# jankammeth/BA-path-planning

Hardware: AMD Instinct MI355X
Metric: SCP iterations/sec (N agents x K waypoints) (higher is better)
Workload: dtype f64

## Files before the change

ba-path-planning_amd/csrc/scp_qp.hip:

```cpp
#include "scp_qp_internal.h"
#include "scp_reset_device.h"

#include <chrono>
#include <cmath>
#include <vector>

__global__ __launch_bounds__(256) void qp_reset_kernel(int N, int K, int D, int Rf, const double* __restrict__ x0,
                                                        const double* __restrict__ F, const double* __restrict__ S0,
                                                        double* __restrict__ x, double* __restrict__ zf,
                                                        double* __restrict__ fx, double* __restrict__ Qx,
                                                        double* __restrict__ yf) {
  extern __shared__ double reset_xs[];
  qp_reset_body<false>(threadIdx.x, true, reset_xs, N, K, D, Rf, x0, F, S0, x, zf, fx, Qx, yf);
}

namespace {

inline size_t align_up(size_t v, size_t a = 256) { return (v + a - 1) / a * a; }

struct Carver {
  char* base;
  size_t off;
  template <typename T>
  T* take(size_t count) {
// ... 46 lines not shown
  d.s0p = c.take<double>(nx);
  d.fx = c.take<double>(nf);
  d.dyf = c.take<double>(nf);
  d.dyc = c.take<double>((size_t)cap);
  const size_t ncell = (size_t)(C / D) * K;
  d.cell_ptr = c.take<int>(ncell + 1);
  d.cell_cur = c.take<int>(ncell);
  d.scan_tot = c.take<int>(ncell / 4096 + 2);
  d.ent_code = c.take<int>((size_t)2 * cap);
  d.coef = c.take<double>((size_t)2 * cap * D);
  d.gval = c.take<double>((size_t)2 * cap);
  d.gval2 = c.take<double>((size_t)2 * cap);
  d.gval3 = c.take<double>((size_t)2 * cap);
  d.pos_i = c.take<int>((size_t)cap);
  d.pos_j = c.take<int>((size_t)cap);
  d.sync_words = c.take<unsigned long long>(SCP_SYNC_WORDS);
  d.cells = c.take<unsigned long long>((size_t)2 * nx);
  d.gpart = c.take<unsigned long long>(SCP_GPART_WORDS);
  d.gcheck = c.take<unsigned long long>(SCP_GCHECK_WORDS);
  return c.off;
}

}

extern "C" void scp_qp_default_settings(scp_qp_settings* s) {
  if (!s) return;
  s->rho = 0.1;
  s->sigma = 1e-6;
  s->alpha = 1.6;
  s->rho_eq_scale = 1e3;
// ... 45 lines not shown
  qp->st = *s;
  qp->row_cap = row_capacity;
  qp->nW = 0;
  qp->problem_set = qp->reset_done = false;
  qp->rho = s->rho;
  carve(qp->d, workspace, K, qp->C, row_capacity, D);
  scp_qp_kkt_init_slots(qp);
  qp->check_seq = 0;
  qp->persist_off = false;
  qp->persist_skip_solve = false;
  qp->persist_gave_up_total = 0;
  qp->persist_variant = 0;
  qp->steps_since_reset = 0;
  memset(qp->lim, 0, sizeof(qp->lim));
  qp->persist_fault = 0;
  qp->persist_cap_nW = -1;
  qp->persist_cap = 0;
  qp->persist_epoch = 0;
  if (hipHostMalloc(&qp->h_scal, (SL_COUNT + SCP_RESID_CAP + 4) * sizeof(double),
                    hipHostMallocMapped | hipHostMallocCoherent) != hipSuccess ||
      hipHostGetDevicePointer((void**)&qp->h_scal_dev, qp->h_scal, 0) != hipSuccess) {
    delete qp;
    return scp_fail(ctx, SCP_ERR_HIP, "qp_create: hipHostMalloc failed");
  }
  memset(qp->h_scal, 0, (SL_COUNT + SCP_RESID_CAP + 4) * sizeof(double));
  qp->h_persist = (unsigned*)(qp->h_scal + SL_COUNT + SCP_RESID_CAP + 1);
  qp->h_persist_dev = (unsigned*)(qp->h_scal_dev + SL_COUNT + SCP_RESID_CAP + 1);
  const int Rf = qp->Rf;
  std::vector<double> F((size_t)Rf * K, 0.0), Ft((size_t)Rf * K, 0.0), S0((size_t)K * K, 0.0), S0t((size_t)K * K, 0.0),
      w(Rf, 1.0);
// ... 406 lines not shown
  if (y_col && qp->nW > 0)
    SCP_HIP_CHECK(ctx, hipMemcpyAsync(y_col, qp->d.yc, qp->nW * sizeof(double), hipMemcpyDeviceToDevice, ctx->stream));
  return SCP_OK;
}

extern "C" int scp_qp_peek(scp_qp* qp, const char* name, double* out, int64_t cap, int64_t* n_out) {
  if (!qp) return SCP_ERR_INVALID;
  scp_ctx* ctx = qp->ctx;
  SCP_REQUIRE(ctx, name && out && n_out, "qp_peek: null pointer");
  const QpDev& d = qp->d;
  const int64_t nf = (int64_t)qp->Rf * qp->C, nx = (int64_t)qp->K * qp->C;
  const double* src = nullptr;
  int64_t n = 0;
  if (!strcmp(name, "fx")) { src = d.fx; n = nf; }
  else if (!strcmp(name, "qx")) { src = scp_qp_qx(qp); n = nx; }
  else if (!strcmp(name, "gval")) { src = d.gval; n = 2 * qp->nW; }
  else if (!strcmp(name, "zf")) { src = d.zf; n = nf; }
  else if (!strcmp(name, "yf")) { src = d.yf; n = nf; }
  else if (!strcmp(name, "zc")) { src = d.zc; n = qp->nW; }
  else if (!strcmp(name, "yc")) { src = d.yc; n = qp->nW; }
  else if (!strcmp(name, "x")) { src = d.x; n = nx; }
  else if (!strcmp(name, "w_eta")) { src = d.w_eta; n = qp->nW * qp->D; }
  else if (!strcmp(name, "w_l")) { src = d.w_l; n = qp->nW; }
  else if (!strcmp(name, "p")) { src = d.p; n = nx; }
  else if (!strcmp(name, "qp")) { src = d.s0p; n = nx; }
  else if (!strcmp(name, "Hf")) { src = d.Hf; n = (int64_t)qp->K * qp->K; }
  else if (!strcmp(name, "Minv")) { src = d.Minv; n = (int64_t)qp->K * qp->K; }
  else if (!strcmp(name, "T")) { src = d.T; n = (int64_t)qp->K * qp->K; }
  else return scp_fail(ctx, SCP_ERR_INVALID, "qp_peek: unknown array %s", name);
  *n_out = n;
  if (n > cap) return scp_fail(ctx, SCP_ERR_CAPACITY, "qp_peek: %lld doubles needed", (long long)n);
  if (n > 0) SCP_HIP_CHECK(ctx, hipMemcpyAsync(out, src, (size_t)n * sizeof(double), hipMemcpyDeviceToDevice, ctx->stream));
  return SCP_OK;
}

extern "C" int scp_qp_debug_set(scp_qp* qp, const char* key, int value) {
  if (!qp || !key) return SCP_ERR_INVALID;
  if (!strcmp(key, "persist_fault")) {
    if (value >= 0) qp->persist_fault = value;
    return qp->persist_fault;
  }
  if (!strcmp(key, "persist_off")) {
    if (value >= 0) qp->persist_off = value != 0;
    return qp->persist_off ? 1 : 0;
  }
  if (!strcmp(key, "persist_gave_up_total")) return qp->persist_gave_up_total;
  return scp_fail(qp->ctx, SCP_ERR_INVALID, "qp_debug_set: unknown key %s", key);
}
```

ba-path-planning_amd/csrc/scp_qp_columns.hip:

```cpp
#include "scp_qp_device.h"

namespace {

using namespace scpdev;
constexpr int FT = 1024;
constexpr int NWV = FT / 64;

#ifdef SCP_PHASE_PROFILE
__device__ unsigned long long scp_phase_clk[64];
#define PHASE_MARK(slot)                                                                      \
  do {                                                                                        \
    if (blockIdx.x == gridDim.x / 2 && threadIdx.x == 0) scp_phase_clk[slot] = wall_clock64(); \
  } while (0)
#else
#define PHASE_MARK(slot) ((void)0)
#endif

constexpr int SQ_BLOCKS = 128;
template <int E>
__global__ __launch_bounds__(FT) void cg1_col_kernel(int K, int Rf, int64_t C, double rho, double h,
                                                      const double* __restrict__ pMinv, const double* __restrict__ wrow,
                                                      const double* __restrict__ x, const double* __restrict__ Fx,
                                                      const double* __restrict__ zf, const double* __restrict__ yf, int N,
                                                      int D, const int* __restrict__ cell_ptr,
// ... 586 lines not shown
  gval[posj] = g;
}

}

int scp_qp_qp0_iterations(scp_qp* qp, int nit, double* dy_out) {
  const QpDev& d = qp->d;
  const int K = qp->K, Rf = qp->Rf;
  const int nblk = (int)((qp->C + CB - 1) / CB);
  const size_t lds = (size_t)CB * (pad_col(Rf) + 3 * pad_col(K)) * sizeof(double);
  return qp_launch(qp, K <= 64 ? qp0_col_kernel<1> : qp0_col_kernel<2>, dim3(nblk), dim3(FT), lds, K, Rf, qp->C, qp->rho,
                   qp->st.sigma, qp->st.alpha, qp->h, nit, d.pMinv, d.wrow, d.lf, d.uf, d.x, d.zf, d.yf, dy_out);
}

int scp_qp_cg1_prepare(scp_qp* qp) {
  if (qp->dv.carried) return SCP_OK;
  QP_CHECK(scp_qp_exact_qx(qp, true));
  QP_CHECK(scp_qp_rows_first_values(qp, scp_qp_qx(qp)));
  qp_on_cg1_prepared(qp);
  return SCP_OK;
}

int scp_qp_cg1_iteration(scp_qp* qp, int* cg_count, bool emit_dy) {
  const QpDev& d = qp->d;
  double* dyf = emit_dy ? d.dyf : nullptr;
  double* dyc = emit_dy ? d.dyc : nullptr;
  const int K = qp->K, Rf = qp->Rf;
  const int64_t C = qp->C;
  const int nblk = (int)((C + CB - 1) / CB);
  double* Qp = d.s0p;
  double* Fp = d.tf;
// ... 314 lines not shown
```

ba-path-planning_amd/csrc/scp_qp_internal.h:

```cpp
#pragma once
#include "scp_common.h"

#define QP_CHECK(call)            \
  do {                            \
    int rc_ = (call);             \
    if (rc_ != SCP_OK) return rc_; \
  } while (0)

constexpr int SCP_KKT_SLOTS = 6;
constexpr int SCP_KKT_SLOTS_MAX = 32;
constexpr size_t SCP_KKT_POOL_BYTES = (size_t)48 << 20;
constexpr int SCP_INV_LDS_MAX_K = 96;
static inline size_t scp_packed_count(int R, int M) { return (size_t)((R + 15) / 16) * ((M + 3) / 4) * 64; }
size_t scp_qp_kkt_pool_doubles(int K);
void scp_qp_kkt_init_slots(scp_qp* qp);
int scp_qp_build_g0(scp_qp* qp);
int scp_qp_build_kkt(scp_qp* qp);

enum Slot {
  SL_RZ0 = 0, SL_RZ1 = 1,
  SL_RP = 8, SL_NAX = 9, SL_NZ = 10, SL_RD = 11, SL_NPX = 12, SL_NATY = 13,
  SL_NDY = 14, SL_SUPP = 15, SL_NATDY = 16,
  SL_COUNT = 32
};
// ... 14 lines not shown
  double* scal;
  double* part;
  double* s0p;
  double* fx;
  double* dyf;
  double* dyc;
  int* cell_ptr;
  int* cell_cur;
  int* scan_tot;
  int* ent_code;
  double* coef;
  double* gval;
  double* gval2;
  double* gval3;
  int *pos_i, *pos_j;
  double* kkt_pool;
  unsigned long long* sync_words;
  unsigned long long* cells;
  unsigned long long* gpart;
  unsigned long long* gcheck;
};

struct QpDerived {
  bool lists = false;
  bool qx = false;
  int qx_half = 0;
  double vals_rho_c = 0.0;
  bool carried = false;
};

struct scp_qp {
  scp_ctx* ctx;
  int N, K, D, Rf;
  int64_t C;
  double h;
  scp_qp_settings st;
  int64_t row_cap, nW;
  bool problem_set, reset_done;
  QpDerived dv;
  double rho;
  QpDev d;
  struct KktSlot {
    double rho, sigma;
    unsigned long long used;
    double *Hf, *HS, *Minv, *T, *pMinv, *pT;
  } kkt[SCP_KKT_SLOTS_MAX];
  int n_kkt;
  unsigned long long kkt_clock;
  double* h_scal;
  double* h_scal_dev;
  unsigned long long check_seq;
  double space[6];
  double lim[6];
  int64_t steps_since_reset;
  int persist_variant;
  int persist_fault;
  bool persist_off;
  bool persist_skip_solve;
  int persist_gave_up_total;
  int64_t persist_cap_nW;
  int persist_cap;
  unsigned long long persist_epoch;
  unsigned* h_persist;
  int persist_rho_switches;
  double persist_rho;
  unsigned* h_persist_dev;
};

constexpr int64_t SCP_FINE_MAX_COLUMNS = 4096;
inline int scp_qp_fine_cadence(const scp_qp* qp) {
  const scp_qp_settings& st = qp->st;
// ... 15 lines not shown
constexpr int NPART = 128;
int scp_qp_generic_iteration(scp_qp* qp, int* cg_count);
int scp_qp_generic_residuals(scp_qp* qp, bool with_dy);
int scp_qp_generic_certificate_atdy(scp_qp* qp);
int scp_qp_exact_qx(scp_qp* qp, bool with_fx);
inline double* scp_qp_qx(const scp_qp* qp, bool other = false) {
  return (qp->dv.qx_half != 0) != other ? qp->d.HQ : qp->d.HQ + (int64_t)qp->K * qp->C;
}

int scp_qp_append_rows(scp_qp* qp, int64_t n, const int64_t* rows, const double* eta, const double* l, int64_t eta_stride,
                       int64_t q_begin, int64_t nq, const double* Qx);
int scp_qp_csr_ensure(scp_qp* qp);
int scp_qp_csr_scatter(scp_qp* qp, int mode, const double* vec);
int scp_qp_rows_gather(scp_qp* qp, const double* Q);
int scp_qp_rows_first_values(scp_qp* qp, const double* Qx);
int scp_qp_rows_check_values(scp_qp* qp, bool with_dy);
int scp_qp_install_rows_small(scp_qp* qp, int64_t n, const int64_t* rows, const double* pos_prev, const double* p0,
                              const double* v0, double R, const double* Qx, bool* done);
int scp_qp_reset_install_small(scp_qp* qp, const double* x0, int64_t n, const int64_t* rows, const double* pos_prev,
                               const double* p0, const double* v0, double R, double* Qx, bool* done);

constexpr int SCP_RESID_STRIDE = 12;
constexpr int SCP_RESID_CAP = (4096 / 2 + 128) * SCP_RESID_STRIDE;
constexpr int SCP_BIGK_MAX_K = 1024;
constexpr int SCP_FUSED_MAX_K = 120;
constexpr int SCP_PART_CAP = 4096;
int scp_qp_cg1_iteration(scp_qp* qp, int* cg_count, bool emit_dy);
int scp_qp_qp0_iterations(scp_qp* qp, int nit, double* dy_out);
int scp_qp_cg1_prepare(scp_qp* qp);
int scp_qp_fused_residuals(scp_qp* qp, bool with_dy);

constexpr int SCP_SYNC_WORDS = 16;
constexpr int SCP_PERSIST_MAX_WG = 256;
constexpr int SCP_GPART_WORDS = 2 * (SCP_PERSIST_MAX_WG + 1) * 4;
constexpr int SCP_GCHECK_WORDS = (SCP_PERSIST_MAX_WG + 1) * 9 * 2;
bool scp_qp_persist_eligible(const scp_qp* qp);
bool scp_persist_claim(int device, int n_cu_total, int n_wg, int wait_ms);
void scp_persist_release(int device, int n_wg);
constexpr int SCP_PERSIST_GAVE_UP = 2;
int scp_qp_cg1_persist(scp_qp* qp, int it0, int cad0, int* ran, int* code, int* it_done);

inline void qp_on_x_set(scp_qp* qp, bool qx) {
  QpDerived& v = qp->dv;
  v.lists = v.carried = false; v.vals_rho_c = 0.0; v.qx = qx;
  if (qx) v.qx_half = 0;
}
inline void qp_on_rows_added(scp_qp* qp, bool small_install) {
  qp->dv.lists = small_install; qp->dv.vals_rho_c = small_install ? qp->rho * qp->st.rho_col_scale : 0.0;
  qp->dv.carried = false;
}
inline void qp_on_rho_changed(scp_qp* qp, bool in_kernel) { qp->dv.vals_rho_c = 0.0; qp->dv.carried &= in_kernel; }
inline void qp_on_solve_start(scp_qp* qp) { qp->dv.carried = false; }
inline void qp_on_scratch_used(scp_qp* qp) { qp->dv.carried = qp->dv.qx = false; qp->dv.vals_rho_c = 0.0; }
inline void qp_on_fused_check(scp_qp* qp) { qp->dv.qx = true; }
inline void qp_on_cg1_step(scp_qp* qp) { qp->dv.qx = false; qp->dv.qx_half ^= 1; }
inline void qp_on_persist_exit(scp_qp* qp, int code) {
  qp->dv.qx = code != SCP_PERSIST_GAVE_UP;
  if (code == SCP_PERSIST_GAVE_UP) qp->dv.carried = false;
}
inline void qp_on_qx_built(scp_qp* qp, bool with_fx) { qp->dv.qx_half = 0; qp->dv.qx = with_fx; }
inline void qp_on_lists_built(scp_qp* qp) { qp->dv.lists = true; }
inline void qp_on_cg1_prepared(scp_qp* qp) { qp->dv.lists = qp->dv.carried = true; qp->dv.vals_rho_c = 0.0; }
```

ba-path-planning_amd/csrc/scp_qp_persist.hip:

```cpp
#include "scp_qp_persist_device.h"

#include <algorithm>
#include <cstdlib>
#include <cerrno>
#include <chrono>


namespace {
using namespace scpdev;
using namespace scp_persist;

#ifdef SCP_PHASE_PROFILE
__device__ unsigned long long scp_persist_clk[16];
#define PSTAMP(slot)                                  \
  do {                                                \
    const unsigned long long now_ = wall_clock64();   \
    pacc[slot] += now_ - plast;                       \
    plast = now_;                                     \
  } while (0)
#else
#define PSTAMP(slot) ((void)0)
#endif

constexpr int persist_apb(int D) { return D == 3 ? 4 : CB / D; }
// ... 28 lines not shown
  int* cptr = e_row + cap;

  const int wave = threadIdx.x >> 6, lane = threadIdx.x & 63;
  const int a0 = blockIdx.x * APB;
  const int agent = a0 + wave;
  const bool aok = agent < N;
  const int k = lane;
  const bool live = aok && k < K;
  const double h = A.h, hh = h * h, alpha = A.alpha;
  double rho = A.rho, rho_c = A.rho_c;
  unsigned n_rho = 0;
  const int tK = (K + 15) >> 4, nks = (K + 3) >> 2;
  const int nblk = A.nblk;

  const int a1 = min(a0 + APB, N);
  const int ebase = A.cell_ptr[cell_of(0, a0, K)];
  const int ne = A.cell_ptr[cell_of(0, a1, K)] - ebase;
  if (entries_overflow<APB>(A)) return;
  if (threadIdx.x == 0) fail_s = 0;
  for (int i = threadIdx.x; i <= (a1 - a0) * K; i += NT) cptr[i] = A.cell_ptr[cell_of(0, a0, K) + i] - ebase;
  for (int e = threadIdx.x; e < ne; e += NT) {
    const int code = A.ent_code[ebase + e];
    const int n = code >> 1, side = code & 1;
    const int wi = A.w_i[n], wj = A.w_j[n], wk = A.w_k[n];
    const int own = side ? wj : wi, par = side ? wi : wj;
    e_code[e] = wk | ((own - a0) << 8) | (side << 16);
    e_pad[e] = ((wk * N + par) * D) * 2;
    e_row[e] = n;
    const int64_t bo = (int64_t)wk * C + (int64_t)own * D, bp = (int64_t)wk * C + (int64_t)par * D;
#pragma unroll
    for (int d = 0; d < D; ++d) {
      const double eta = A.w_eta[(size_t)n * D + d];
      e_c[(size_t)e * D + d] = side ? -eta : eta;
      e_qo[(size_t)e * D + d] = A.Qx[bo + d];
      e_qp[(size_t)e * D + d] = A.Qx[bp + d];
    }
    e_l[e] = A.w_l[n];
    e_z[e] = A.zc[n];
    e_y[e] = A.yc[n];
    e_g[e] = A.gval[ebase + e];
  }
  for (int i = threadIdx.x; i < CB * RSK; i += NT) Rt[i] = 0.0;

  double z[D][4], y[D][4], lo[D][4], hi[D][4], fx[D][4], rr[4], x[D], qx[D];
#pragma unroll
  for (int t = 0; t < 4; ++t) {
    const bool rok = live && (t > 0 || k < K - 1);
    const int row = t == 0 ? k : t * K - 1 + k;
    rr[t] = (t >= 2 && k == K - 1) ? rho * A.rho_eq : rho;
#pragma unroll
    for (int d = 0; d < D; ++d) {
      z[d][t] = y[d][t] = lo[d][t] = hi[d][t] = fx[d][t] = 0.0;
      if (rok) {
        const int64_t g = (int64_t)row * C + (int64_t)agent * D + d;
        z[d][t] = A.zf[g]; y[d][t] = A.yf[g]; lo[d][t] = A.lf[g]; hi[d][t] = A.uf[g]; fx[d][t] = A.fx[g];
// ... 353 lines not shown
        A.zf[g] = z[d][t];
        A.yf[g] = y[d][t];
        A.fx[g] = fx[d][t];
        if (with_dy) A.dyf[g] = dy[d][t];
      }
    }
  }
  if (live) {
#pragma unroll
    for (int d = 0; d < D; ++d) {
      const int64_t g = (int64_t)k * C + (int64_t)agent * D + d;
      A.x[g] = x[d];
      A.Qx[g] = qx[d];
    }
  }
  for (int e = threadIdx.x; e < ne; e += NT) {
    A.gval[ebase + e] = e_g[e];
    if (!((e_code[e] >> 16) & 1)) {
      A.zc[e_row[e]] = e_z[e];
      A.yc[e_row[e]] = e_y[e];
      if (with_dy) A.dyc[e_row[e]] = e_pp[(size_t)e * D];
    }
  }
  PSTAMP(8);
#ifdef SCP_PHASE_PROFILE
  if (blockIdx.x == gridDim.x / 2 && threadIdx.x == 0)
    for (int i = 0; i < 16; ++i) scp_persist_clk[i] = i == 15 ? (unsigned long long)steps : pacc[i];
#endif
  publish_exit(A, chk, it_done, n_rho, rho, exit_code);
}

size_t persist_lds_bytes(int K, int cap, int nblk, int D, int apb) {
  size_t dbl = (size_t)3 * CB * pad_col(K) + (size_t)apb * 64 * D + (size_t)NCHK * nblk + (size_t)cap * (4 * D + 4);
  size_t ints = (size_t)3 * cap + (size_t)apb * K + 1;
  return dbl * sizeof(double) + ((ints + 1) / 2 * 2) * sizeof(int);
// ... 36 lines not shown
}

int scp_qp_cg1_persist(scp_qp* qp, int it0, int cad0, int* ran, int* code, int* it_done) {
  const QpDev& d = qp->d;
  scp_ctx* ctx = qp->ctx;
  hipStream_t s = ctx->stream;
  const scp_qp_settings& st = qp->st;
  const int K = qp->K, D = qp->D;
  const int64_t C = qp->C;
  const int variant = persist_variant_for(qp);
  if (variant < 0) { *ran = 0; return SCP_OK; }
  const PersistKernel pk = persist_kernel(variant, D);
  const int apb = pk.apb;
  const int nblk = (qp->N + apb - 1) / apb;
  *ran = 0;
  QP_CHECK(scp_qp_cg1_prepare(qp));
  if (qp->persist_cap_nW == qp->nW) return SCP_OK;
  {
    const int nb = nblk + 1;
    const size_t fixed = pk.lds_bytes(K, 0, nb, D, apb);
    const size_t budget_lds = 160 * 1024 - pk.static_lds;
    if (fixed + 64 * pk.entry_bytes > budget_lds) return SCP_OK;
    qp->persist_cap = (int)((budget_lds - fixed) / pk.entry_bytes / 64 * 64);
  }
  const int nblk_expected = nblk + (qp->persist_fault > 0 ? 1 : 0);
  const size_t lds = pk.lds_bytes(K, qp->persist_cap, nblk_expected, D, apb);
  if (lds > 160 * 1024) return SCP_OK;
  const int budget = st.max_iter - it0;
  if (budget <= 0) return SCP_OK;
  if (!scp_persist_claim(ctx->device, ctx->n_cu, nblk, 200)) {
    qp->persist_skip_solve = true;
    return SCP_OK;
  }
  if (qp->persist_fault > 0) --qp->persist_fault;
  struct ClaimGuard {
    int device, n;
    ~ClaimGuard() { scp_persist_release(device, n); }
  } claim_guard{ctx->device, nblk};
// ... 19 lines not shown
    }();
    a.spin_sleep = spin_sleep;
  }
  a.rho_tol = (st.adaptive_rho && st.adaptive_rho_interval > 0) ? st.adaptive_rho_tolerance : 0.0;
  a.pMinv = d.pMinv;
  a.pT = d.pT;
  a.lf = d.lf; a.uf = d.uf; a.zf = d.zf; a.yf = d.yf; a.fx = d.fx; a.x = d.x;
  a.Qx = scp_qp_qx(qp);
  a.dyf = d.dyf;
  a.cells = d.cells;
  a.gpart = d.gpart;
  a.gcheck = d.gcheck;
  a.give_up = (unsigned*)d.sync_words;
  a.cell_ptr = d.cell_ptr; a.ent_code = d.ent_code; a.w_k = d.w_k; a.w_i = d.w_i; a.w_j = d.w_j;
  a.w_eta = d.w_eta; a.w_l = d.w_l; a.zc = d.zc; a.yc = d.yc; a.dyc = d.dyc; a.gval = d.gval;
  a.host_status = qp->h_persist_dev;
  a.host_scal = qp->h_scal_dev;
  a.host_flag = (u64*)(qp->h_scal_dev + SL_COUNT + SCP_RESID_CAP);
  a.host_rho = qp->h_scal_dev + SL_COUNT + SCP_RESID_CAP + 3;
  a.rho_col_scale = st.rho_col_scale;
  a.n_tab = 0;
  for (int i = 0; i < qp->n_kkt; ++i)
    if (qp->kkt[i].used && qp->kkt[i].sigma == st.sigma) {
      a.tab[a.n_tab].rho = qp->kkt[i].rho;
      a.tab[a.n_tab].pMinv = qp->kkt[i].pMinv;
      a.tab[a.n_tab].pT = qp->kkt[i].pT;
      ++a.n_tab;
    }
  a.seq = ++qp->check_seq;
  qp->h_persist[0] = 0u;
// ... 16 lines not shown
  SCP_HIP_CHECK(ctx, hipGetLastError());
  *ran = 1;
  {
    volatile u64* flag = (volatile u64*)(qp->h_scal + SL_COUNT + SCP_RESID_CAP);
    if (!scp_wait_host_word(flag, a.seq, 30)) SCP_HIP_CHECK(ctx, hipStreamSynchronize(s));
    if (*flag != a.seq) return scp_fail(ctx, SCP_ERR_HIP, "persistent kernel: completion word not written");
    __atomic_thread_fence(__ATOMIC_ACQUIRE);
  }
  *code = (int)((volatile unsigned*)qp->h_persist)[0];
  *it_done = (int)((volatile unsigned*)qp->h_persist)[1];
  if (*code == EXIT_OVERFLOW) {
    qp->persist_cap_nW = qp->nW;
    *ran = 0;
    return SCP_OK;
  }
  qp_on_persist_exit(qp, *code);
  if (*code == SCP_PERSIST_GAVE_UP) {
    ++qp->persist_gave_up_total;
  } else {
    qp->persist_epoch += (u64)(*it_done - it0);
    qp->persist_rho_switches = (int)((volatile unsigned*)qp->h_persist)[2];
    qp->persist_rho = ((volatile double*)qp->h_scal)[SL_COUNT + SCP_RESID_CAP + 3];
  }
  return SCP_OK;
}

#include <fcntl.h>
#include <signal.h>
#include <sys/mman.h>
#include <time.h>
#include <unistd.h>
// ... 110 lines not shown
```

ba-path-planning_amd/csrc/scp_qp_persist16.hip:

```cpp
#include "scp_qp_persist_device.h"

namespace {
using namespace scpdev;
using namespace scp_persist;

#ifdef SCP_PHASE_PROFILE
__device__ unsigned long long scp_persist16_clk[16];
#define PSTAMP(slot)                                           \
  do {                                                         \
    if (prof_t) {                                              \
      const unsigned long long now_ = wall_clock64();          \
      pacc_s[slot] += now_ - pacc_s[15];                       \
      pacc_s[15] = now_;                                       \
    }                                                          \
  } while (0)
#else
#define PSTAMP(slot) ((void)0)
#endif

constexpr int nct_of(int D, int APB) { return (D * APB + 15) / 16; }
constexpr int AB_STRIDE = 32;

constexpr bool t_on_mfma(int D, int APB) { return 4 * nct_of(D, APB) < APB && APB <= 8; }
constexpr int ent_doubles(int D) { return D + 6; }
// ... 69 lines not shown
  int* cptr = e_code + cap;

  const int wave = threadIdx.x >> 6, lane = threadIdx.x & 63;
  const int a0 = blockIdx.x * APB16;
  const int agent = a0 + wave;
  const bool aok = agent < N;
  const int k = lane;
  const bool live = aok && k < K;
  const bool jok = live && k < K - 1;
  const bool lastk = k == K - 1;
  const double h = A.h, hh = h * h, ih = 1.0 / h, alpha = A.alpha;
  double rho = A.rho, rho_c = A.rho_c;
  unsigned n_rho = 0;

  const int a1 = min(a0 + APB16, N);
  const int ebase = A.cell_ptr[cell_of(0, a0, K)];
  const int ne = A.cell_ptr[cell_of(0, a1, K)] - ebase;
  if (entries_overflow<APB16>(A)) return;
  if (threadIdx.x == 0) fail_s = 0;
  for (int i = threadIdx.x; i <= (a1 - a0) * K; i += NT16) cptr[i] = A.cell_ptr[cell_of(0, a0, K) + i] - ebase;
  for (int e = threadIdx.x; e < ne; e += NT16) {
    const int code = A.ent_code[ebase + e];
    const int n = code >> 1, side = code & 1;
    const int wi = A.w_i[n], wj = A.w_j[n], wk = A.w_k[n];
    const int own = side ? wj : wi, par = side ? wi : wj;
    e_code[e] = wk | ((own - a0) << 6) | (side << 10) | (par << 11);
    const int64_t bo = (int64_t)wk * C + (int64_t)own * D, bp = (int64_t)wk * C + (int64_t)par * D;
    double ax = 0.0;
#pragma unroll
    for (int d = 0; d < D; ++d) {
      const double eta = A.w_eta[(size_t)n * D + d];
      const double c = side ? -eta : eta;
      e_c[(size_t)e * D + d] = c;
      ax += c * (A.Qx[bo + d] - A.Qx[bp + d]);
    }
    e_ax[e] = ax;
    e_l[e] = A.w_l[n];
    e_z[e] = A.zc[n];
    e_y[e] = A.yc[n];
    e_g[e] = A.gval[ebase + e];
  }
  for (int i = threadIdx.x; i < NC16 * RSK; i += NT16) Rt[i] = 0.0;
  for (int i = threadIdx.x; i < tK * nks * 64; i += NT16) {
    Ml[i] = A.pMinv[i];
    if constexpr (TQ) Tl[i] = A.pT[i];
  }

  double v[D][4], off[D], x[D], c1[D], c2[D];
#pragma unroll
  for (int t = 0; t < 4; ++t) {
    const bool rok = t == 0 ? jok : live;
    const int row = t == 0 ? k : t * K - 1 + k;
    const double rr = (t >= 2 && lastk) ? rho * A.rho_eq : rho;
#pragma unroll
    for (int d = 0; d < D; ++d) {
// ... 454 lines not shown
    for (int t = 0; t < 4; ++t) {
      if (t == 0 ? jok : live) {
        const int row = t == 0 ? k : t * K - 1 + k;
        const int64_t g = (int64_t)row * C + (int64_t)agent * D + d;
        A.zf[g] = zc[t];
        A.yf[g] = ((t >= 2 && lastk) ? rho * A.rho_eq : rho) * (v[d][t] - zc[t]);
        A.fx[g] = f[t];
      }
    }
    if (live) {
      const int64_t g = (int64_t)k * C + (int64_t)agent * D + d;
      A.x[g] = x[d];
      A.Qx[g] = hh * (c2[d] - 0.5 * c1b);
    }
  }
  for (int e = threadIdx.x; e < ne; e += NT16) {
    A.gval[ebase + e] = e_g[e];
    if (!((e_code[e] >> 10) & 1)) {
      const int n = A.ent_code[ebase + e] >> 1;
      A.zc[n] = e_z[e];
      A.yc[n] = e_y[e];
    }
  }
  PSTAMP(8);
#ifdef SCP_PHASE_PROFILE
  if (prof_t)
    for (int i = 0; i < 16; ++i) scp_persist16_clk[i] = i == 15 ? (unsigned long long)steps : pacc_s[i];
#endif
  publish_exit(A, chk_s, it_done, n_rho, rho, exit_code);
}

}

#ifdef SCP_PHASE_PROFILE
extern "C" int scp_debug_persist16_clocks(unsigned long long* out, int n) {
  if (n > 16) n = 16;
// ... 19 lines not shown
```

ba-path-planning_amd/csrc/scp_qp_persist_device.h:

```cpp
#pragma once
#include "scp_qp_device.h"

#if defined(__HIP_DEVICE_COMPILE__) && !defined(__gfx950__)
#error "scp_qp_persist_device.h: the persistent ADMM kernels' hand-offs are written for gfx950 only"
#endif

namespace scp_persist {
using namespace scpdev;

typedef unsigned long long u64;
constexpr unsigned SPIN_LIMIT = 1u << 20;

struct PersistArgs {
  int K, N, nblk, ent_cap;
  int it0, max_iter, check_every, rho_interval;
  int cad0, check_fine;
  double fine_ratio;
  int64_t C;
  double rho, rho_c, rho_eq, alpha, h;
  double eps_abs, eps_rel, eps_prim_inf, rho_tol;
  double jerk_lo, jerk_hi, acc_lo, acc_hi, vel_lo, vel_hi, pmin[3], pmax[3];
  const double* states;
  int first_step;
  int spin_sleep;
  const double* pMinv;
  const double* pT;
  const double *lf, *uf;
  double *zf, *yf, *fx, *x, *Qx, *dyf;
  u64* cells;
  u64* gpart;
  u64* gcheck;
  unsigned* give_up;
  const int *cell_ptr, *ent_code, *w_k, *w_i, *w_j;
  const double *w_eta, *w_l;
  double *zc, *yc, *dyc, *gval;
  unsigned* host_status;
  double* host_scal;
  u64* host_flag;
  u64 seq;
  unsigned epoch0;
  double rho_col_scale;
  double* host_rho;
  int n_tab;
  struct RhoSlot {
    double rho;
    const double* pMinv;
    const double* pT;
  } tab[SCP_KKT_SLOTS_MAX];
};

// ... 120 lines not shown
    if (cand > rho * A.rho_tol * (1.0 - 1e-9) || cand < rho / A.rho_tol * (1.0 + 1e-9)) {
      int s = -1;
      for (int i = 0; i < A.n_tab; ++i)
        if (fabs(A.tab[i].rho - cand) <= 1e-12 * cand) s = i;
      if (s < 0) return EXIT_RHO;
      const double nrs = A.tab[s].rho;
      if (nrs > rho * A.rho_tol || nrs < rho / A.rho_tol) {
        slot = s;
        if (A.check_fine > 0) cad = A.check_fine;
      }
    }
  }
  return 0;
}

template <int APB>
__device__ __forceinline__ bool entries_overflow(const PersistArgs& A) {
  int worst = 0;
  for (int b = threadIdx.x; b < (A.N + APB - 1) / APB; b += 64 * APB) {
    const int b0 = b * APB, b1 = min(b0 + APB, A.N);
    worst = max(worst, A.cell_ptr[cell_of(0, b1, A.K)] - A.cell_ptr[cell_of(0, b0, A.K)]);
  }
  if (!__syncthreads_or(worst > A.ent_cap)) return false;
  if (blockIdx.x == 0 && threadIdx.x == 0) {
    __hip_atomic_store(A.host_status, (unsigned)EXIT_OVERFLOW, __ATOMIC_RELAXED, __HIP_MEMORY_SCOPE_SYSTEM);
    __hip_atomic_store(A.host_flag, A.seq, __ATOMIC_RELEASE, __HIP_MEMORY_SCOPE_SYSTEM);
  }
  return true;
}

__device__ __forceinline__ bool leave_if_gave_up(const PersistArgs& A, bool ok) {
  if (ok && __syncthreads_or(threadIdx.x == 0 &&
                             __hip_atomic_load(A.give_up, __ATOMIC_RELAXED, __HIP_MEMORY_SCOPE_AGENT) != 0u))
    ok = false;
  if (ok) return false;
  if (threadIdx.x == 0) {
    __hip_atomic_store(A.host_status, (unsigned)EXIT_GAVE_UP, __ATOMIC_RELAXED, __HIP_MEMORY_SCOPE_SYSTEM);
    __hip_atomic_store(A.host_flag, A.seq, __ATOMIC_RELEASE, __HIP_MEMORY_SCOPE_SYSTEM);
  }
  return true;
}

__device__ __forceinline__ void publish_exit(const PersistArgs& A, const double* chk, int it_done, unsigned n_rho, double rho,
// ... 21 lines not shown
```

ba-path-planning_amd/csrc/scp_qp_rows.hip:

```cpp
#include "scp_qp_device.h"
#include "scp_pair_device.h"
#include "scp_reset_device.h"

#include <algorithm>

__global__ __launch_bounds__(256) void add_rows_kernel(int N, int D, int64_t C, int64_t pairs, int64_t base, int64_t n,
                                                        const int64_t* __restrict__ rows,
                                                        const double* __restrict__ eta_in,
                                                        const double* __restrict__ l_in, int64_t eta_stride,
                                                        int64_t q_begin, int64_t nq, const double* __restrict__ Q,
                                                        int64_t* __restrict__ w_row, int* __restrict__ wk,
                                                        int* __restrict__ wi, int* __restrict__ wj,
                                                        double* __restrict__ weta, double* __restrict__ wl,
                                                        double* __restrict__ zc, double* __restrict__ yc) {
  const int64_t t = (int64_t)blockIdx.x * 256 + threadIdx.x;
  if (t >= n) return;
  const int64_t r = rows[t];
  const int64_t k = r / pairs, q = r % pairs;
  const double b = 2.0 * N - 1.0;
  int64_t ii = (int64_t)((b - sqrt(b * b - 8.0 * (double)q)) * 0.5);
  if (ii < 0) ii = 0;
  if (ii > N - 2) ii = N - 2;
  while (ii * (2LL * N - ii - 1) / 2 > q) --ii;
  while (ii < N - 2 && (ii + 1) * (2LL * N - ii - 2) / 2 <= q) ++ii;
// ... 393 lines not shown
    QP_CHECK(qp_launch(qp, csr_finish_kernel, grid1(2 * qp->nW), b256, 0, 2 * qp->nW, qp->D, d.ent_code, d.w_eta, d.coef, d.pos_i,
                       d.pos_j));
  }
  qp_on_lists_built(qp);
  return SCP_OK;
}

int scp_qp_csr_scatter(scp_qp* qp, int mode, const double* vec) {
  QP_CHECK(scp_qp_csr_ensure(qp));
  const QpDev& d = qp->d;
  QP_CHECK(qp_launch(qp, csr_rowval_kernel, grid1(qp->nW), dim3(256), 0, qp->nW, mode, qp->rho * qp->st.rho_col_scale, d.zc, d.yc,
                     vec, d.pos_i, d.pos_j, d.gval, nullptr, nullptr));
  return launch_gather(qp);
}

int scp_qp_rows_check_values(scp_qp* qp, bool with_dy) {
  const QpDev& d = qp->d;
  return qp_launch(qp, csr_rowval_kernel, grid1(qp->nW), dim3(256), 0, qp->nW, 1, 0.0, d.zc, d.yc, nullptr, d.pos_i, d.pos_j,
                   d.gval2, with_dy ? d.dyc : nullptr, with_dy ? d.gval3 : nullptr);
}

int scp_qp_rows_gather(scp_qp* qp, const double* Q) {
  const QpDev& d = qp->d;
  QP_CHECK(scp_qp_csr_ensure(qp));
  QP_CHECK(qp_launch(qp, qp->D == 2 ? rows_value_kernel<2, false> : rows_value_kernel<3, false>, grid1(qp->nW), dim3(256), 0,
                     qp->nW, qp->C, qp->rho * qp->st.rho_col_scale, d.w_k, d.w_i, d.w_j, d.w_eta, Q, d.zc, d.yc, d.pos_i,
                     d.pos_j, d.gval));
  return launch_gather(qp);
}
```

Before: 415.5.

## Build per-block constraint entry tables inside persistent kernel instead of host CSR

When no CSR lists exist, each persistent workgroup scans the constraint row list itself, bins its own entries by cell in LDS, prefix-scans the cell counts and insertion-sorts within cells, which skips the separate CSR build kernels and the prepare pass. Row values are carried per row in a new grow buffer and converted back to entry order only when another path needs them. This adds a full scan of all rows per block and LDS atomics inside the kernel, and caps the entry capacity.

```diff
diff --git a/ba-path-planning_amd/csrc/scp_qp.hip b/ba-path-planning_amd/csrc/scp_qp.hip
--- a/ba-path-planning_amd/csrc/scp_qp.hip
+++ b/ba-path-planning_amd/csrc/scp_qp.hip
@@ -84,6 +84,8 @@
   d.gval3 = c.take<double>((size_t)2 * cap);
   d.pos_i = c.take<int>((size_t)cap);
   d.pos_j = c.take<int>((size_t)cap);
+  d.grow = c.take<double>((size_t)cap);
+  d.own_code = c.take<int>((size_t)(SCP_PERSIST_MAX_WG + 1) * SCP_PERSIST_CAP_MAX);
   d.sync_words = c.take<unsigned long long>(SCP_SYNC_WORDS);
   d.cells = c.take<unsigned long long>((size_t)2 * nx);
   d.gpart = c.take<unsigned long long>(SCP_GPART_WORDS);
@@ -159,6 +161,10 @@
   qp->steps_since_reset = 0;
   memset(qp->lim, 0, sizeof(qp->lim));
   qp->persist_fault = 0;
+  {
+    const char* e = getenv("SCP_PERSIST_HOST_LISTS");
+    qp->persist_host_lists = e && atoi(e) != 0;
+  }
   qp->persist_cap_nW = -1;
   qp->persist_cap = 0;
   qp->persist_epoch = 0;
@@ -595,7 +601,10 @@
   int64_t n = 0;
   if (!strcmp(name, "fx")) { src = d.fx; n = nf; }
   else if (!strcmp(name, "qx")) { src = scp_qp_qx(qp); n = nx; }
-  else if (!strcmp(name, "gval")) { src = d.gval; n = 2 * qp->nW; }
+  else if (!strcmp(name, "gval")) {
+    if (qp->dv.carried && qp->dv.vals_by_row) QP_CHECK(scp_qp_rows_values_to_entries(qp));
+    src = d.gval; n = 2 * qp->nW;
+  }
   else if (!strcmp(name, "zf")) { src = d.zf; n = nf; }
   else if (!strcmp(name, "yf")) { src = d.yf; n = nf; }
   else if (!strcmp(name, "zc")) { src = d.zc; n = qp->nW; }
@@ -621,6 +630,10 @@
     if (value >= 0) qp->persist_fault = value;
     return qp->persist_fault;
   }
+  if (!strcmp(key, "persist_host_lists")) {
+    if (value >= 0) qp->persist_host_lists = value != 0;
+    return qp->persist_host_lists ? 1 : 0;
+  }
   if (!strcmp(key, "persist_off")) {
     if (value >= 0) qp->persist_off = value != 0;
     return qp->persist_off ? 1 : 0;
diff --git a/ba-path-planning_amd/csrc/scp_qp_columns.hip b/ba-path-planning_amd/csrc/scp_qp_columns.hip
--- a/ba-path-planning_amd/csrc/scp_qp_columns.hip
+++ b/ba-path-planning_amd/csrc/scp_qp_columns.hip
@@ -624,7 +624,8 @@
 }
 
 int scp_qp_cg1_prepare(scp_qp* qp) {
-  if (qp->dv.carried) return SCP_OK;
+  if (qp->dv.carried)
+    return qp->dv.vals_by_row ? scp_qp_rows_values_to_entries(qp) : SCP_OK;
   QP_CHECK(scp_qp_exact_qx(qp, true));
   QP_CHECK(scp_qp_rows_first_values(qp, scp_qp_qx(qp)));
   qp_on_cg1_prepared(qp);
diff --git a/ba-path-planning_amd/csrc/scp_qp_internal.h b/ba-path-planning_amd/csrc/scp_qp_internal.h
--- a/ba-path-planning_amd/csrc/scp_qp_internal.h
+++ b/ba-path-planning_amd/csrc/scp_qp_internal.h
@@ -52,6 +52,8 @@
   double* gval2;
   double* gval3;
   int *pos_i, *pos_j;
+  double* grow;
+  int* own_code;
   double* kkt_pool;
   unsigned long long* sync_words;
   unsigned long long* cells;
@@ -65,6 +67,7 @@
   int qx_half = 0;
   double vals_rho_c = 0.0;
   bool carried = false;
+  bool vals_by_row = false;
 };
 
 struct scp_qp {
@@ -93,6 +96,7 @@
   int64_t steps_since_reset;
   int persist_variant;
   int persist_fault;
+  bool persist_host_lists;
   bool persist_off;
   bool persist_skip_solve;
   int persist_gave_up_total;
@@ -138,6 +142,7 @@
 int scp_qp_csr_scatter(scp_qp* qp, int mode, const double* vec);
 int scp_qp_rows_gather(scp_qp* qp, const double* Q);
 int scp_qp_rows_first_values(scp_qp* qp, const double* Qx);
+int scp_qp_rows_values_to_entries(scp_qp* qp);
 int scp_qp_rows_check_values(scp_qp* qp, bool with_dy);
 int scp_qp_install_rows_small(scp_qp* qp, int64_t n, const int64_t* rows, const double* pos_prev, const double* p0,
                               const double* v0, double R, const double* Qx, bool* done);
@@ -156,6 +161,7 @@
 
 constexpr int SCP_SYNC_WORDS = 16;
 constexpr int SCP_PERSIST_MAX_WG = 256;
+constexpr int SCP_PERSIST_CAP_MAX = 2432;
 constexpr int SCP_GPART_WORDS = 2 * (SCP_PERSIST_MAX_WG + 1) * 4;
 constexpr int SCP_GCHECK_WORDS = (SCP_PERSIST_MAX_WG + 1) * 9 * 2;
 bool scp_qp_persist_eligible(const scp_qp* qp);
@@ -178,10 +184,14 @@
 inline void qp_on_scratch_used(scp_qp* qp) { qp->dv.carried = qp->dv.qx = false; qp->dv.vals_rho_c = 0.0; }
 inline void qp_on_fused_check(scp_qp* qp) { qp->dv.qx = true; }
 inline void qp_on_cg1_step(scp_qp* qp) { qp->dv.qx = false; qp->dv.qx_half ^= 1; }
-inline void qp_on_persist_exit(scp_qp* qp, int code) {
+inline void qp_on_persist_exit(scp_qp* qp, int code, bool own_lists) {
   qp->dv.qx = code != SCP_PERSIST_GAVE_UP;
   if (code == SCP_PERSIST_GAVE_UP) qp->dv.carried = false;
+  else if (own_lists) qp->dv.carried = qp->dv.vals_by_row = true;
 }
 inline void qp_on_qx_built(scp_qp* qp, bool with_fx) { qp->dv.qx_half = 0; qp->dv.qx = with_fx; }
 inline void qp_on_lists_built(scp_qp* qp) { qp->dv.lists = true; }
-inline void qp_on_cg1_prepared(scp_qp* qp) { qp->dv.lists = qp->dv.carried = true; qp->dv.vals_rho_c = 0.0; }
+inline void qp_on_cg1_prepared(scp_qp* qp) {
+  qp->dv.lists = qp->dv.carried = true; qp->dv.vals_by_row = false; qp->dv.vals_rho_c = 0.0;
+}
+inline void qp_on_vals_to_entries(scp_qp* qp) { qp->dv.vals_by_row = false; }
diff --git a/ba-path-planning_amd/csrc/scp_qp_persist.hip b/ba-path-planning_amd/csrc/scp_qp_persist.hip
--- a/ba-path-planning_amd/csrc/scp_qp_persist.hip
+++ b/ba-path-planning_amd/csrc/scp_qp_persist.hip
@@ -66,13 +66,20 @@
   const int nblk = A.nblk;
 
   const int a1 = min(a0 + APB, N);
-  const int ebase = A.cell_ptr[cell_of(0, a0, K)];
-  const int ne = A.cell_ptr[cell_of(0, a1, K)] - ebase;
-  if (entries_overflow<APB>(A)) return;
+  int ebase0 = 0, ne;
+  if (A.own_lists) {
+    ne = build_entry_tables<APB, NT>(A, a0, a1, cptr, e_code, (int*)e_pp, (int*)Rt, (int*)gp);
+    if (ne < 0) return;
+  } else {
+    ebase0 = A.cell_ptr[cell_of(0, a0, K)];
+    ne = A.cell_ptr[cell_of(0, a1, K)] - ebase0;
+    if (entries_overflow<APB>(A)) return;
+    for (int i = threadIdx.x; i <= (a1 - a0) * K; i += NT) cptr[i] = A.cell_ptr[cell_of(0, a0, K) + i] - ebase0;
+  }
   if (threadIdx.x == 0) fail_s = 0;
-  for (int i = threadIdx.x; i <= (a1 - a0) * K; i += NT) cptr[i] = A.cell_ptr[cell_of(0, a0, K) + i] - ebase;
   for (int e = threadIdx.x; e < ne; e += NT) {
-    const int code = A.ent_code[ebase + e];
+    const bool own_lists = A.own_lists != 0;
+    const int code = own_lists ? e_code[e] : A.ent_code[ebase0 + e];
     const int n = code >> 1, side = code & 1;
     const int wi = A.w_i[n], wj = A.w_j[n], wk = A.w_k[n];
     const int own = side ? wj : wi, par = side ? wi : wj;
@@ -80,17 +87,21 @@
     e_pad[e] = ((wk * N + par) * D) * 2;
     e_row[e] = n;
     const int64_t bo = (int64_t)wk * C + (int64_t)own * D, bp = (int64_t)wk * C + (int64_t)par * D;
+    double ax = 0.0;
 #pragma unroll
     for (int d = 0; d < D; ++d) {
       const double eta = A.w_eta[(size_t)n * D + d];
-      e_c[(size_t)e * D + d] = side ? -eta : eta;
-      e_qo[(size_t)e * D + d] = A.Qx[bo + d];
-      e_qp[(size_t)e * D + d] = A.Qx[bp + d];
+      const double c = side ? -eta : eta, qo = A.Qx[bo + d], qp = A.Qx[bp + d];
+      e_c[(size_t)e * D + d] = c;
+      e_qo[(size_t)e * D + d] = qo;
+      e_qp[(size_t)e * D + d] = qp;
+      ax = __builtin_fma(c, qo - qp, ax);
     }
     e_l[e] = A.w_l[n];
-    e_z[e] = A.zc[n];
-    e_y[e] = A.yc[n];
-    e_g[e] = A.gval[ebase + e];
+    const double zc = A.zc[n], yc = A.yc[n];
+    e_z[e] = zc;
+    e_y[e] = yc;
+    e_g[e] = !own_lists ? A.gval[ebase0 + e] : (A.vals_carried ? A.grow[n] : first_row_value(rho_c, zc, yc, ax));
   }
   for (int i = threadIdx.x; i < CB * RSK; i += NT) Rt[i] = 0.0;
 
@@ -474,11 +485,14 @@
       A.Qx[g] = qx[d];
     }
   }
+  const bool own_lists = A.own_lists != 0;
+  const int ebase = own_lists ? 0 : A.cell_ptr[cell_of(0, a0, K)];
   for (int e = threadIdx.x; e < ne; e += NT) {
-    A.gval[ebase + e] = e_g[e];
+    if (!own_lists) A.gval[ebase + e] = e_g[e];
     if (!((e_code[e] >> 16) & 1)) {
       A.zc[e_row[e]] = e_z[e];
       A.yc[e_row[e]] = e_y[e];
+      if (own_lists) A.grow[e_row[e]] = e_g[e];
       if (with_dy) A.dyc[e_row[e]] = e_pp[(size_t)e * D];
     }
   }
@@ -545,14 +559,16 @@
   const int apb = pk.apb;
   const int nblk = (qp->N + apb - 1) / apb;
   *ran = 0;
-  QP_CHECK(scp_qp_cg1_prepare(qp));
+  const bool own_lists = !qp->persist_host_lists && !qp->dv.lists && qp->nW < (1 << 29);
+  if (!own_lists) QP_CHECK(scp_qp_cg1_prepare(qp));
+  else if (!qp->dv.carried) QP_CHECK(scp_qp_exact_qx(qp, true));
   if (qp->persist_cap_nW == qp->nW) return SCP_OK;
   {
     const int nb = nblk + 1;
     const size_t fixed = pk.lds_bytes(K, 0, nb, D, apb);
     const size_t budget_lds = 160 * 1024 - pk.static_lds;
     if (fixed + 64 * pk.entry_bytes > budget_lds) return SCP_OK;
-    qp->persist_cap = (int)((budget_lds - fixed) / pk.entry_bytes / 64 * 64);
+    qp->persist_cap = std::min((int)((budget_lds - fixed) / pk.entry_bytes / 64 * 64), SCP_PERSIST_CAP_MAX);
   }
   const int nblk_expected = nblk + (qp->persist_fault > 0 ? 1 : 0);
   const size_t lds = pk.lds_bytes(K, qp->persist_cap, nblk_expected, D, apb);
@@ -602,6 +618,8 @@
   a.give_up = (unsigned*)d.sync_words;
   a.cell_ptr = d.cell_ptr; a.ent_code = d.ent_code; a.w_k = d.w_k; a.w_i = d.w_i; a.w_j = d.w_j;
   a.w_eta = d.w_eta; a.w_l = d.w_l; a.zc = d.zc; a.yc = d.yc; a.dyc = d.dyc; a.gval = d.gval;
+  a.nW = (int)qp->nW; a.own_lists = own_lists ? 1 : 0; a.own_code = d.own_code; a.grow = d.grow;
+  a.vals_carried = own_lists && qp->dv.carried ? 1 : 0;
   a.host_status = qp->h_persist_dev;
   a.host_scal = qp->h_scal_dev;
   a.host_flag = (u64*)(qp->h_scal_dev + SL_COUNT + SCP_RESID_CAP);
@@ -648,7 +666,7 @@
     *ran = 0;
     return SCP_OK;
   }
-  qp_on_persist_exit(qp, *code);
+  qp_on_persist_exit(qp, *code, own_lists);
   if (*code == SCP_PERSIST_GAVE_UP) {
     ++qp->persist_gave_up_total;
   } else {
diff --git a/ba-path-planning_amd/csrc/scp_qp_persist16.hip b/ba-path-planning_amd/csrc/scp_qp_persist16.hip
--- a/ba-path-planning_amd/csrc/scp_qp_persist16.hip
+++ b/ba-path-planning_amd/csrc/scp_qp_persist16.hip
@@ -107,13 +107,21 @@
   unsigned n_rho = 0;
 
   const int a1 = min(a0 + APB16, N);
-  const int ebase = A.cell_ptr[cell_of(0, a0, K)];
-  const int ne = A.cell_ptr[cell_of(0, a1, K)] - ebase;
-  if (entries_overflow<APB16>(A)) return;
+  int ebase0 = 0, ne;
+  if (A.own_lists) {
+    ne = build_entry_tables<APB16, NT16>(A, a0, a1, cptr, e_code, (int*)e_s, (int*)Rt, (int*)gp);
+    if (ne < 0) return;
+  } else {
+    ebase0 = A.cell_ptr[cell_of(0, a0, K)];
+    ne = A.cell_ptr[cell_of(0, a1, K)] - ebase0;
+    if (entries_overflow<APB16>(A)) return;
+    for (int i = threadIdx.x; i <= (a1 - a0) * K; i += NT16) cptr[i] = A.cell_ptr[cell_of(0, a0, K) + i] - ebase0;
+  }
   if (threadIdx.x == 0) fail_s = 0;
-  for (int i = threadIdx.x; i <= (a1 - a0) * K; i += NT16) cptr[i] = A.cell_ptr[cell_of(0, a0, K) + i] - ebase;
   for (int e = threadIdx.x; e < ne; e += NT16) {
-    const int code = A.ent_code[ebase + e];
+    const bool own_lists = A.own_lists != 0;
+    const int code = own_lists ? e_code[e] : A.ent_code[ebase0 + e];
+    if (own_lists) A.own_code[(size_t)blockIdx.x * cap + e] = code;
     const int n = code >> 1, side = code & 1;
     const int wi = A.w_i[n], wj = A.w_j[n], wk = A.w_k[n];
     const int own = side ? wj : wi, par = side ? wi : wj;
@@ -129,9 +137,10 @@
     }
     e_ax[e] = ax;
     e_l[e] = A.w_l[n];
-    e_z[e] = A.zc[n];
-    e_y[e] = A.yc[n];
-    e_g[e] = A.gval[ebase + e];
+    const double zc = A.zc[n], yc = A.yc[n];
+    e_z[e] = zc;
+    e_y[e] = yc;
+    e_g[e] = !own_lists ? A.gval[ebase0 + e] : (A.vals_carried ? A.grow[n] : first_row_value(rho_c, zc, yc, ax));
   }
   for (int i = threadIdx.x; i < NC16 * RSK; i += NT16) Rt[i] = 0.0;
   for (int i = threadIdx.x; i < tK * nks * 64; i += NT16) {
@@ -616,12 +625,15 @@
       A.Qx[g] = hh * (c2[d] - 0.5 * c1b);
     }
   }
+  const bool own_lists = A.own_lists != 0;
+  const int ebase = own_lists ? 0 : A.cell_ptr[cell_of(0, a0, K)];
   for (int e = threadIdx.x; e < ne; e += NT16) {
-    A.gval[ebase + e] = e_g[e];
+    if (!own_lists) A.gval[ebase + e] = e_g[e];
     if (!((e_code[e] >> 10) & 1)) {
-      const int n = A.ent_code[ebase + e] >> 1;
+      const int n = (own_lists ? A.own_code[(size_t)blockIdx.x * cap + e] : A.ent_code[ebase + e]) >> 1;
       A.zc[n] = e_z[e];
       A.yc[n] = e_y[e];
+      if (own_lists) A.grow[n] = e_g[e];
     }
   }
   PSTAMP(8);
diff --git a/ba-path-planning_amd/csrc/scp_qp_persist_device.h b/ba-path-planning_amd/csrc/scp_qp_persist_device.h
--- a/ba-path-planning_amd/csrc/scp_qp_persist_device.h
+++ b/ba-path-planning_amd/csrc/scp_qp_persist_device.h
@@ -34,6 +34,9 @@
   const int *cell_ptr, *ent_code, *w_k, *w_i, *w_j;
   const double *w_eta, *w_l;
   double *zc, *yc, *dyc, *gval;
+  int nW, own_lists, vals_carried;
+  int* own_code;
+  double* grow;
   unsigned* host_status;
   double* host_scal;
   u64* host_flag;
@@ -184,6 +187,14 @@
   return 0;
 }
 
+__device__ __forceinline__ bool leave_on_overflow(const PersistArgs& A, bool over) {
+  if (!__syncthreads_or(over)) return false;
+  if (blockIdx.x == 0 && threadIdx.x == 0) {
+    __hip_atomic_store(A.host_status, (unsigned)EXIT_OVERFLOW, __ATOMIC_RELAXED, __HIP_MEMORY_SCOPE_SYSTEM);
+    __hip_atomic_store(A.host_flag, A.seq, __ATOMIC_RELEASE, __HIP_MEMORY_SCOPE_SYSTEM);
+  }
+  return true;
+}
 template <int APB>
 __device__ __forceinline__ bool entries_overflow(const PersistArgs& A) {
   int worst = 0;
@@ -191,12 +202,100 @@
     const int b0 = b * APB, b1 = min(b0 + APB, A.N);
     worst = max(worst, A.cell_ptr[cell_of(0, b1, A.K)] - A.cell_ptr[cell_of(0, b0, A.K)]);
   }
-  if (!__syncthreads_or(worst > A.ent_cap)) return false;
-  if (blockIdx.x == 0 && threadIdx.x == 0) {
-    __hip_atomic_store(A.host_status, (unsigned)EXIT_OVERFLOW, __ATOMIC_RELAXED, __HIP_MEMORY_SCOPE_SYSTEM);
-    __hip_atomic_store(A.host_flag, A.seq, __ATOMIC_RELEASE, __HIP_MEMORY_SCOPE_SYSTEM);
-  }
-  return true;
+  return leave_on_overflow(A, worst > A.ent_cap);
+}
+
+template <int APB, int NT>
+__device__ __forceinline__ int build_entry_tables(const PersistArgs& A, int a0, int a1, int* cptr, int* codes, int* hits,
+                                                  int* cur, int* blk_cnt) {
+  static_assert(APB <= 16 && (APB & (APB - 1)) == 0, "one wave scans 64 x 16 cells; blocks by shift");
+  const int K = A.K, nW = A.nW, cap = A.ent_cap, tid = threadIdx.x, me = blockIdx.x;
+  const int nb = (A.N + APB - 1) / APB, ncell = (a1 - a0) * K;
+  for (int i = tid; i <= ncell; i += NT) cptr[i] = 0;
+  for (int i = tid; i < ncell; i += NT) cur[i] = 0;
+  for (int i = tid; i < nb; i += NT) blk_cnt[i] = 0;
+  __syncthreads();
+  constexpr int U = 4;
+  for (int n0 = tid; n0 < nW; n0 += U * NT) {
+    int w[U][2];
+#pragma unroll
+    for (int u = 0; u < U; ++u) {
+      const int n = n0 + u * NT;
+      w[u][0] = n < nW ? A.w_i[n] : -1;
+      w[u][1] = n < nW ? A.w_j[n] : -1;
+    }
+#pragma unroll
+    for (int u = 0; u < U; ++u) {
+      const int n = n0 + u * NT;
+#pragma unroll
+      for (int side = 0; side < 2; ++side) {
+        const int ag = w[u][side];
+        if (ag < 0) continue;
+        if (ag / APB != me) {
+          atomicAdd(&blk_cnt[ag / APB], 1);
+        } else {
+          const int at = atomicAdd(&blk_cnt[me], 1);
+          const int cell = (ag - a0) * K + A.w_k[n];
+          atomicAdd(&cptr[cell], 1);
+          if (at < cap) {
+            hits[2 * at] = 2 * n + side;
+            hits[2 * at + 1] = cell;
+          }
+        }
+      }
+    }
+  }
+  __syncthreads();
+  int worst = 0;
+  for (int b = tid; b < nb; b += NT) worst = max(worst, blk_cnt[b]);
+  if (leave_on_overflow(A, worst > cap)) return -1;
+  const int ne = blk_cnt[me];
+  if (tid < 64) {
+    constexpr int SC = 16;
+    int v[SC], tot = 0;
+#pragma unroll
+    for (int e = 0; e < SC; ++e) {
+      v[e] = SC * tid + e < ncell ? cptr[SC * tid + e] : 0;
+      tot += v[e];
+    }
+    int incl = tot;
+#pragma unroll
+    for (int o = 1; o < 64; o <<= 1) {
+      const int t = __shfl_up(incl, o);
+      if (tid >= o) incl += t;
+    }
+    int run = incl - tot;
+#pragma unroll
+    for (int e = 0; e < SC; ++e) {
+      if (SC * tid + e < ncell) cptr[SC * tid + e] = run;
+      run += v[e];
+    }
+    if (tid == 63) cptr[ncell] = run;
+  }
+  __syncthreads();
+  for (int t = tid; t < ne; t += NT) {
+    const int cell = hits[2 * t + 1];
+    codes[cptr[cell] + atomicAdd(&cur[cell], 1)] = hits[2 * t];
+  }
+  __syncthreads();
+  for (int c = tid; c < ncell; c += NT) {
+    const int b = cptr[c], e = cptr[c + 1];
+    for (int i = b + 1; i < e; ++i) {
+      const int v = codes[i];
+      int j = i - 1;
+      while (j >= b && codes[j] > v) {
+        codes[j + 1] = codes[j];
+        --j;
+      }
+      codes[j + 1] = v;
+    }
+  }
+  __syncthreads();
+  return ne;
+}
+
+__device__ __forceinline__ double first_row_value(double rho_c, double zc, double yc, double ax) {
+  return __builtin_fma(-rho_c, ax, __builtin_fma(rho_c, zc, -yc));
 }
 
 __device__ __forceinline__ bool leave_if_gave_up(const PersistArgs& A, bool ok) {
diff --git a/ba-path-planning_amd/csrc/scp_qp_rows.hip b/ba-path-planning_amd/csrc/scp_qp_rows.hip
--- a/ba-path-planning_amd/csrc/scp_qp_rows.hip
+++ b/ba-path-planning_amd/csrc/scp_qp_rows.hip
@@ -431,6 +431,15 @@
   return launch_gather(qp);
 }
 
+int scp_qp_rows_values_to_entries(scp_qp* qp) {
+  const QpDev& d = qp->d;
+  QP_CHECK(scp_qp_csr_ensure(qp));
+  QP_CHECK(qp_launch(qp, csr_rowval_kernel, grid1(qp->nW), dim3(256), 0, qp->nW, 2, 0.0, d.zc, d.yc, d.grow, d.pos_i, d.pos_j,
+                     d.gval, nullptr, nullptr));
+  qp_on_vals_to_entries(qp);
+  return SCP_OK;
+}
+
 int scp_qp_rows_check_values(scp_qp* qp, bool with_dy) {
   const QpDev& d = qp->d;
   return qp_launch(qp, csr_rowval_kernel, grid1(qp->nW), dim3(256), 0, qp->nW, 1, 0.0, d.zc, d.yc, nullptr, d.pos_i, d.pos_j,
```

After: 423.5 (median of 6 runs). About the same (+1.9%).
